# google-deepmind/mujoco_warp

Measured on AMD Instinct MI355X. Metric: env-steps/sec (nworld x steps/s) for humanoid.xml at 8192 worlds, 1/2/4/8 GPUs, higher is better.
Workload: dtype f32; 1 GPU; humanoid.xml, nworld=8192 per GPU, CG solver, Euler, pyramidal, nconmax=24, njmax=64, key 0 + Halton/OU control noise (std 0.01, rate 0.1); nworld_per_gpu=8192, nworld_total=8192, parallelism=worlds sharded over 1 GPU(s), no data-path collective

## Files before the change

### mujoco_warp_amd/csrc/solver_cgp.hpp

```cpp
#pragma once
#include <type_traits>
#include "solver.hpp"
#include "solver_cgw.hpp"

#ifndef MJH_CGP_HOIST
#define MJH_CGP_HOIST 1
#endif
#define CGP_HEAD 32
#define CGP_WORLD 136
template <int NV4>
__host__ __device__ inline int cgp_pool_rows(size_t lds_bytes, int wpb) {
  constexpr int NVR = 4 * NV4, JS = (NV4 & 1) ? NVR : NVR + 4;
  const int words = (int)(lds_bytes / sizeof(float)) - CGP_HEAD - CGP_WORLD * wpb;
  return words <= 0 ? 0 : ((words / JS) & ~3);
}
template <int NV4>
__host__ __device__ inline int cgp_min_rows(int fuse_euler) {
  constexpr int NVR = 4 * NV4, JS = (NV4 & 1) ? NVR : NVR + 4;
  const int words = fuse_euler == 2 ? (6 * 32 + 12 * NV4 + 4 + 32) : (8 * NVR > 32 ? 8 * NVR : 32);
  return (((words + JS - 1) / JS) + 3) & ~3;
}

template <int CTRL>
DEV float qperm(float v) {
  return __int_as_float(__builtin_amdgcn_mov_dpp(__float_as_int(v), CTRL, 0xf, 0xf, true));
}
template <int C>
DEV void fmac_rbc(float& acc, float a, float xs) {
  asm volatile("v_fmac_f32_dpp %0, %1, %2 row_newbcast:%3 row_mask:0xf bank_mask:0xf bound_ctrl:1" : "+v"(acc) : "v"(xs), "v"(a), "n"(C));
}
DEV void dpp_fence(BV& x) { asm volatile("s_nop 4" : "+v"(x.a), "+v"(x.b)); }
template <int C>
DEV void fmac4_rbc(float& s0, float& s1, float a0, float a1, float a2, float a3, float xs) {
  asm volatile(
      "v_fmac_f32_dpp %0, %2, %3 row_newbcast:%7 row_mask:0xf bank_mask:0xf bound_ctrl:1\n\t"
      "v_fmac_f32_dpp %1, %2, %4 row_newbcast:%8 row_mask:0xf bank_mask:0xf bound_ctrl:1\n\t"
      "v_fmac_f32_dpp %0, %2, %5 row_newbcast:%9 row_mask:0xf bank_mask:0xf bound_ctrl:1\n\t"
      "v_fmac_f32_dpp %1, %2, %6 row_newbcast:%10 row_mask:0xf bank_mask:0xf bound_ctrl:1"
      : "+v"(s0), "+v"(s1)
      : "v"(xs), "v"(a0), "v"(a1), "v"(a2), "v"(a3), "n"(C), "n"(C + 1), "n"(C + 2), "n"(C + 3));
}
template <int OFF, int N, int NT>
DEV void fmac_seq(float (&s)[2], const float (&row)[N], float xs) {
  static_assert(NT % 4 == 0, "four terms per asm statement");
  if constexpr (NT >= 4) fmac4_rbc<0>(s[0], s[1], row[OFF], row[OFF + 1], row[OFF + 2], row[OFF + 3], xs);
  if constexpr (NT >= 8) fmac4_rbc<4>(s[0], s[1], row[OFF + 4], row[OFF + 5], row[OFF + 6], row[OFF + 7], xs);
  if constexpr (NT >= 12) fmac4_rbc<8>(s[0], s[1], row[OFF + 8], row[OFF + 9], row[OFF + 10], row[OFF + 11], xs);
  if constexpr (NT >= 16) fmac4_rbc<12>(s[0], s[1], row[OFF + 12], row[OFF + 13], row[OFF + 14], row[OFF + 15], xs);
}
template <int N, int NT>
DEV void fmac_seq2(float (&s)[4], const float (&r0)[N], const float (&r1)[N], float xs) {
  static_assert(NT % 4 == 0, "four terms per asm statement");
  if constexpr (NT >= 4) { fmac4_rbc<0>(s[0], s[1], r0[0], r0[1], r0[2], r0[3], xs); fmac4_rbc<0>(s[2], s[3], r1[0], r1[1], r1[2], r1[3], xs); }
  if constexpr (NT >= 8) { fmac4_rbc<4>(s[0], s[1], r0[4], r0[5], r0[6], r0[7], xs); fmac4_rbc<4>(s[2], s[3], r1[4], r1[5], r1[6], r1[7], xs); }
  if constexpr (NT >= 12) { fmac4_rbc<8>(s[0], s[1], r0[8], r0[9], r0[10], r0[11], xs); fmac4_rbc<8>(s[2], s[3], r1[8], r1[9], r1[10], r1[11], xs); }
  if constexpr (NT >= 16) { fmac4_rbc<12>(s[0], s[1], r0[12], r0[13], r0[14], r0[15], xs); fmac4_rbc<12>(s[2], s[3], r1[12], r1[13], r1[14], r1[15], xs); }
}

template <int NVR, int G>
DEV void invert_rows_b4s(const float (&mrow)[NVR], float (&s)[NVR], float* buf, int lig) {
#pragma unroll
  for (int c = 0; c < NVR; ++c) s[c] = mrow[c];
#pragma unroll
  for (int kb = 0; kb < NVR / 4; ++kb) {
    constexpr int T = 4 * NVR;
    const int k = 4 * kb;
    float* pb = buf + (kb & 1) * T;
    const int q = lig - k;
    if (q >= 0 && q < 4) {
#pragma unroll
      for (int c4 = 0; c4 < NVR / 4; ++c4) *reinterpret_cast<float4*>(pb + q * NVR + 4 * c4) = make_float4(s[4 * c4], s[4 * c4 + 1], s[4 * c4 + 2], s[4 * c4 + 3]);
    }
    gsync();
    const float4 P0 = *reinterpret_cast<const float4*>(pb + k), P1 = *reinterpret_cast<const float4*>(pb + NVR + k),
                 P2 = *reinterpret_cast<const float4*>(pb + 2 * NVR + k), P3 = *reinterpret_cast<const float4*>(pb + 3 * NVR + k);
    const float i0 = 1.0f / P0.x;
    const float l10 = P1.x * i0, l20 = P2.x * i0, l30 = P3.x * i0;
    const float i1 = 1.0f / (P1.y - l10 * P1.x);
    const float t21 = P2.y - l20 * P1.x, t31 = P3.y - l30 * P1.x;
    const float l21 = t21 * i1, l31 = t31 * i1;
    const float i2 = 1.0f / (P2.z - l20 * P2.x - l21 * t21);
    const float t32 = P3.z - l30 * P2.x - l31 * t21;
    const float l32 = t32 * i2;
    const float i3 = 1.0f / (P3.w - l30 * P3.x - l31 * t31 - l32 * t32);
    const float n10 = -l10, n21 = -l21, n32 = -l32;
    const float n20 = -l20 - l21 * n10, n31 = -l31 - l32 * n21;
    const float n30 = -l30 - l31 * n10 - l32 * n20;
    const float e30 = i3 * n30, e31 = i3 * n31, e32 = i3 * n32, e20 = i2 * n20, e21 = i2 * n21, e10 = i1 * n10;
    float Pi[4][4];
    Pi[3][3] = i3;
    Pi[2][3] = Pi[3][2] = e32;
    Pi[1][3] = Pi[3][1] = e31;
    Pi[0][3] = Pi[3][0] = e30;
    Pi[2][2] = i2 + n32 * e32;
    Pi[1][2] = Pi[2][1] = e21 + n31 * e32;
    Pi[0][2] = Pi[2][0] = e20 + n30 * e32;
    Pi[1][1] = i1 + n21 * e21 + n31 * e31;
    Pi[0][1] = Pi[1][0] = e10 + n20 * e21 + n30 * e31;
    Pi[0][0] = i0 + n10 * e10 + n20 * e20 + n30 * e30;
    const bool inb = q >= 0 && q < 4;
    float F[4];
#pragma unroll
    for (int p = 0; p < 4; ++p) {
      const float out = s[k] * Pi[0][p] + s[k + 1] * Pi[1][p] + s[k + 2] * Pi[2][p] + s[k + 3] * Pi[3][p];
      const float own = (q == p ? 1.0f : 0.0f) - (q == 0 ? Pi[0][p] : (q == 1 ? Pi[1][p] : (q == 2 ? Pi[2][p] : Pi[3][p])));
      F[p] = inb ? own : out;
    }
#pragma unroll
    for (int c4 = 0; c4 < NVR / 4; ++c4) {
      if (c4 == kb) continue;
      const float4 r0 = *reinterpret_cast<const float4*>(pb + 4 * c4), r1 = *reinterpret_cast<const float4*>(pb + NVR + 4 * c4),
                   r2 = *reinterpret_cast<const float4*>(pb + 2 * NVR + 4 * c4), r3 = *reinterpret_cast<const float4*>(pb + 3 * NVR + 4 * c4);
      s[4 * c4] -= F[0] * r0.x + F[1] * r1.x + F[2] * r2.x + F[3] * r3.x;
      s[4 * c4 + 1] -= F[0] * r0.y + F[1] * r1.y + F[2] * r2.y + F[3] * r3.y;
      s[4 * c4 + 2] -= F[0] * r0.z + F[1] * r1.z + F[2] * r2.z + F[3] * r3.z;
      s[4 * c4 + 3] -= F[0] * r0.w + F[1] * r1.w + F[2] * r2.w + F[3] * r3.w;
    }
#pragma unroll
    for (int e = 0; e < 4; ++e) s[k + e] = (q == e ? 1.0f : 0.0f) - F[e];
  }
}

template <int NV4>
DEV void solve_cgp_body(const MjhModel& m, const MjhData& d, float* smem, int slot0, int nwb, int pool_rows, int fuse_euler) {
  constexpr int G = 32, NR = 2, NVR = 4 * NV4, JS = (NV4 & 1) ? NVR : NVR + 4, J4 = JS / 4;
  constexpr int NA = NVR < 16 ? NVR : 16, NBX = NVR - NA;
  const int nv = m.nv, nC = m.nC, njmax = d.njmax, nvp = d.nv_pad;
  const int lig = threadIdx.x & (G - 1), gib = threadIdx.x / G;
  const int slot = slot0 + gib;
  const bool valid = gib < nwb && slot < d.nworld;
  int* cnt = reinterpret_cast<int*>(smem);
  int* slotR = reinterpret_cast<int*>(smem) + CGP_HEAD + CGP_WORLD * gib;
  float* fbT = smem + CGP_HEAD + CGP_WORLD * gib + 64;
  float* pool = smem + CGP_HEAD + CGP_WORLD * (blockDim.x / G);
  const bool active = lig < nv;

  const int w = valid ? d.ws_order[slot] : 0;
  const size_t vo = (size_t)w * nv, eo = (size_t)w * njmax;
  int idx[NVR];
  {
    const int nv4r = (nv + 3) >> 2;
    const int4* tab = reinterpret_cast<const int4*>(m.M_dense) + (size_t)(active ? lig : 0) * nv4r;
#pragma unroll
    for (int c4 = 0; c4 < NV4; ++c4) {
      const int4 t4 = c4 < nv4r ? tab[c4] : make_int4(-1, -1, -1, -1);
      idx[4 * c4] = t4.x; idx[4 * c4 + 1] = t4.y; idx[4 * c4 + 2] = t4.z; idx[4 * c4 + 3] = t4.w;
    }
  }
  int nefc = 0, ne = 0, nf = 0, npf = 0;
  int ty[2] = {0, 0};
  if (valid) {
    nefc = min(d.nefc[w], njmax);
    ne = d.ne[w];
    nf = d.nf[w];
    npf = ne + nf + d.nl[w];
#pragma unroll
    for (int k = 0; k < 2; ++k) ty[k] = lig + G * k < njmax ? d.efc_type[eo + lig + G * k] : 0;
  }
  float mrow[NVR];
  {
    const float* Mg = d.M + (size_t)w * nC;
#pragma unroll
    for (int c = 0; c < NVR; ++c) {
      const float v = Mg[idx[c] < 0 ? 0 : idx[c]];
      mrow[c] = active ? (idx[c] < 0 ? 0.0f : v) : (c == lig ? 1.0f : 0.0f);
    }
  }
  const float fs = active ? d.qfrc_smooth[vo + lig] : 0.0f;
  const float qwarm = active ? d.qacc_warmstart[vo + lig] : 0.0f;

  int np = 0, nq = 0, need = 0;
  bool defer = false;
  if (valid) {
    npf = min(npf, nefc);
    bool is6[2];
#pragma unroll
    for (int k = 0; k < 2; ++k) {
      const int r = lig + G * k;
      is6[k] = r >= npf && r < nefc && ty[k] == CT_CONTACT_PYRAMIDAL;
    }
    const unsigned m0 = (unsigned)gballot<G>(is6[0]), m1 = (unsigned)gballot<G>(is6[1]);
    const int n60 = __popc(m0), n6 = n60 + __popc(m1);
    const unsigned below = (1u << lig) - 1u;
#pragma unroll
    for (int k = 0; k < 2; ++k) {
      const int r = lig + G * k;
      const int c6 = k == 0 ? __popc(m0 & below) : n60 + __popc(m1 & below);
      if (r < nefc && r < 64) slotR[is6[k] ? c6 : n6 + r - c6] = r;
      fbT[r] = 0.0f;
    }
    nq = n6 >> 2;
    np = nefc - n6;
    defer = nf > 0 || (n6 & 3) != 0 || nefc > 64;
    need = max((np + 3 * nq + 15) & ~15, cgp_min_rows<NV4>(fuse_euler));
  }
  if (lig == 0 && gib < CGP_HEAD) cnt[gib] = (valid && !defer) ? need : 0;
  __syncthreads();
  int base = 0;
  {
    int acc = 0;
    for (int j = 0; j < nwb; ++j) {
      const int c = cnt[j];
      const bool fits = acc + c <= pool_rows;
      if (j == gib) {
        base = acc;
        if (!fits) defer = true;
      }
      acc += fits ? c : 0;
    }
  }
  if (!valid) return;
  if (defer) {
    if (lig == 0) d.solver_niter[w] = -1;
    return;
  }
  float* Jl = pool + (size_t)base * JS;
  const int nb = np + 3 * nq, nb16 = (nb + 15) & ~15;

  PhaseClock pc(5, lig);
  pc.mark(0);
  const bool warm = !(m.disableflags & DSBL_WARMSTART);
  auto mul_row = [&](const float (&row)[NVR], BV x) __attribute__((always_inline)) {
    float s[2] = {0.0f, 0.0f};
    dpp_fence(x);
    fmac_seq<0, NVR, NA>(s, row, x.a);
    if constexpr (NBX > 0) fmac_seq<NA, NVR, NBX>(s, row, x.b);
    return active ? s[0] + s[1] : 0.0f;
  };
  float h[NVR];
  invert_rows_b4s<NVR, G>(mrow, h, Jl, lig);
  float qs = mul_row(h, bcast_prep(fs));
  {
    const float res = fs - mul_row(mrow, bcast_prep(qs));
    qs += mul_row(h, bcast_prep(active ? res : 0.0f));
  }
  if (active) d.qacc_smooth[vo + lig] = qs;
  float q = active ? (nefc > 0 && warm ? qwarm : qs) : 0.0f;
  pc.mark(1);
  float Ma = mul_row(mrow, bcast_prep(q));
  if (nefc == 0) {
    if (active) {
      d.qacc[vo + lig] = q;
      d.qfrc_constraint[vo + lig] = 0.0f;
      d.efc_Ma[vo + lig] = Ma;
    }
    if (lig == 0) d.solver_niter[w] = 0;
    if (fuse_euler) {
      float qi = q;
      gsync();
      if (fuse_euler == 2) qi = impfast_acc<NV4, G>(m, d, w, lig, active, mrow, Ma, Jl);
      euler_advance<G>(m, d, w, lig, active, qi, Jl + (fuse_euler == 2 ? 6 * G + 12 * NV4 + 4 : 0), q);
    }
    return;
  }

  float rD[NR], rja[NR], rjv[NR];
  int rkind[NR];
  int jro[NR];
  int fbo[NR];
  bool isq[NR];
  int rer[NR];
  const int qd = lig & 3;
#pragma unroll
  for (int k = 0; k < NR; ++k) {
    const int s = lig + G * k;
    const bool has = s < nefc;
    isq[k] = s < 4 * nq;
    const int er = has ? slotR[s] : 0;
    rer[k] = er;
    const int br = isq[k] ? 3 * (s >> 2) + (qd < 3 ? qd : 2) : (has ? s - nq : 0);
    const int bf_ = isq[k] ? (qd < 3 ? 3 * (s >> 2) + qd : -1) : s - nq;
    jro[k] = br * JS;
    fbo[k] = (!has || bf_ < 0) ? 64 : bf_;
    rD[k] = has ? d.efc_D[eo + er] : 0.0f;
    rkind[k] = !has ? 3 : (isq[k] ? 2 : (er < ne ? 0 : 2));
    rjv[k] = 0.0f;
    rja[k] = has ? d.efc_aref[eo + er] : 0.0f;
  }
  gsync();
  {
    const float* Jg = d.efc_J + (size_t)w * d.njmax_pad * nvp;
    const int nvp4 = nvp >> 2;
    for (int it = lig; it < nq * J4; it += G) {
      const int c = it / J4, c4 = it - c * J4;
      float4 r0 = make_float4(0.0f, 0.0f, 0.0f, 0.0f), r1 = r0, r2 = r0, r3 = r0;
      if (c4 < nvp4) {
        const float4* src = reinterpret_cast<const float4*>(Jg + (size_t)slotR[4 * c] * nvp) + c4;
        r0 = src[0]; r1 = src[nvp4]; r2 = src[2 * nvp4]; r3 = src[3 * nvp4];
      }
      float4* dst = reinterpret_cast<float4*>(Jl + (size_t)(3 * c) * JS) + c4;
      dst[0] = make_float4(0.5f * (r0.x + r1.x), 0.5f * (r0.y + r1.y), 0.5f * (r0.z + r1.z), 0.5f * (r0.w + r1.w));
      dst[J4] = make_float4(0.5f * (r0.x - r1.x), 0.5f * (r0.y - r1.y), 0.5f * (r0.z - r1.z), 0.5f * (r0.w - r1.w));
      dst[2 * J4] = make_float4(0.5f * (r2.x - r3.x), 0.5f * (r2.y - r3.y), 0.5f * (r2.z - r3.z), 0.5f * (r2.w - r3.w));
    }
    for (int it = lig; it < (nb16 - 3 * nq) * J4; it += G) {
      const int p = it / J4, c4 = it - p * J4;
      float4 v = make_float4(0.0f, 0.0f, 0.0f, 0.0f);
      if (p < np && c4 < nvp4) v = (reinterpret_cast<const float4*>(Jg + (size_t)slotR[4 * nq + p] * nvp))[c4];
      (reinterpret_cast<float4*>(Jl + (size_t)(3 * nq + p) * JS))[c4] = v;
    }
  }
  gsync();
  auto j_dots = [&](auto nxt, BV x, float (&out)[NR], float* mv) __attribute__((always_inline)) {
    constexpr int NX = decltype(nxt)::value;
    float s[4] = {0.0f, 0.0f, 0.0f, 0.0f};
    float r0[NA], r1[NA];
    auto load_a = [&]() __attribute__((always_inline)) {
#pragma unroll
      for (int c4 = 0; c4 < NA / 4; ++c4) {
        const float4 a4 = *reinterpret_cast<const float4*>(Jl + jro[0] + 4 * c4);
        r0[4 * c4] = a4.x; r0[4 * c4 + 1] = a4.y; r0[4 * c4 + 2] = a4.z; r0[4 * c4 + 3] = a4.w;
        if constexpr (NX > 1) {
          const float4 b4 = *reinterpret_cast<const float4*>(Jl + jro[1] + 4 * c4);
          r1[4 * c4] = b4.x; r1[4 * c4 + 1] = b4.y; r1[4 * c4 + 2] = b4.z; r1[4 * c4 + 3] = b4.w;
        }
      }
    };
    if constexpr (NV4 <= 7) load_a();
    dpp_fence(x);
    if (mv) {
      float t[2] = {0.0f, 0.0f};
      fmac_seq<0, NVR, NA>(t, mrow, x.a);
      if constexpr (NBX > 0) fmac_seq<NA, NVR, NBX>(t, mrow, x.b);
      *mv = active ? t[0] + t[1] : 0.0f;
    }
    if constexpr (NV4 > 7) load_a();
    constexpr int NB_ = NBX > 0 ? NBX : 4;
    float q0[NB_], q1[NB_];
    if constexpr (NBX > 0) {
#pragma unroll
      for (int c4 = 0; c4 < NBX / 4; ++c4) {
        const float4 a4 = *reinterpret_cast<const float4*>(Jl + jro[0] + NA + 4 * c4);
        q0[4 * c4] = a4.x; q0[4 * c4 + 1] = a4.y; q0[4 * c4 + 2] = a4.z; q0[4 * c4 + 3] = a4.w;
        if constexpr (NX > 1) {
          const float4 b4 = *reinterpret_cast<const float4*>(Jl + jro[1] + NA + 4 * c4);
          q1[4 * c4] = b4.x; q1[4 * c4 + 1] = b4.y; q1[4 * c4 + 2] = b4.z; q1[4 * c4 + 3] = b4.w;
        }
      }
    }
    if constexpr (NX > 1) {
      fmac_seq2<NA, NA>(s, r0, r1, x.a);
      if constexpr (NBX > 0) fmac_seq2<NB_, NBX>(s, q0, q1, x.b);
    } else {
      float s2[2] = {0.0f, 0.0f};
      fmac_seq<0, NA, NA>(s2, r0, x.a);
      if constexpr (NBX > 0) fmac_seq<0, NB_, NBX>(s2, q0, x.b);
      s[0] = s2[0];
      s[1] = s2[1];
    }
#pragma unroll
    for (int k = 0; k < NR; ++k) {
      if (k >= NX) {
        out[k] = 0.0f;
        continue;
      }
      const float dt = s[2 * k] + s[2 * k + 1];
      const float dn = qperm<0x00>(dt), d1 = qperm<0x55>(dt), d2 = qperm<0xAA>(dt);
      const float tq = qd < 2 ? d1 : d2;
      const float dq = dn + ((qd & 1) ? -tq : tq);
      out[k] = rkind[k] == 3 ? 0.0f : (isq[k] ? dq : dt);
    }
  };
  {
    float jq[NR];
    j_dots(std::integral_constant<int, NR>{}, bcast_prep(q), jq, nullptr);
#pragma unroll
    for (int k = 0; k < NR; ++k) rja[k] = rkind[k] != 3 ? jq[k] - rja[k] : 0.0f;
  }
  pc.mark(2);
  const float tolerance = bf(m.opt_tolerance, m.opt_tolerance_nb, w, 1)[0];
  const float ls_tolerance = bf(m.opt_ls_tolerance, m.opt_ls_tolerance_nb, w, 1)[0];
  const float meaninertia = bf(m.stat_meaninertia, m.stat_meaninertia_nb, w, 1)[0];
  const float scale = meaninertia * (float)nv;
  const float rscale = 1.0f / scale;
  const int qd4 = lig >> 2;
  const int cq = qd4 < J4 ? qd4 : (qd4 - 4 >= 0 && qd4 - 4 < J4 ? qd4 - 4 : J4 - 1), rg = lig & 3;
  const float* Jq = Jl + 4 * cq + 4 * rg * JS;
  const float *Jq1 = Jq + min(16, nb16 - 16) * JS, *Jq2 = Jq + min(32, nb16 - 16) * JS, *Jq3 = Jq + min(48, nb16 - 16) * JS;

  float grad_dot = 0.0f, search_dot = 0.0f;
  float g = 0.0f, Mg = 0.0f, pg = 0.0f, pMg = 0.0f, srch = 0.0f, qc = 0.0f;
  float cg5[5] = {0.0f, 0.0f, 0.0f, 0.0f, 0.0f};
  int niter = 0;
  const int maxiter = m.iterations, ls_iterations = m.ls_iterations;
  int ovf = 0;
  float improvement = 0.0f;
  const bool short16 = __ballot(nb16 > 16) == 0ull;
  auto iterate = [&](auto nxt) __attribute__((always_inline)) {
  constexpr int NX = decltype(nxt)::value;
  for (;;) {
#if MJH_CGP_HOIST
    const float4 hj0 = *reinterpret_cast<const float4*>(Jq), hj1 = *reinterpret_cast<const float4*>(Jq + JS),
                 hj2 = *reinterpret_cast<const float4*>(Jq + 2 * JS), hj3 = *reinterpret_cast<const float4*>(Jq + 3 * JS);
#endif
#if MJH_CGP_HOIST > 1
    float4 gj0 = make_float4(0.0f, 0.0f, 0.0f, 0.0f), gj1 = gj0, gj2 = gj0, gj3 = gj0;
    if (!(NX == 1 && short16)) {
      gj0 = *reinterpret_cast<const float4*>(Jq1); gj1 = *reinterpret_cast<const float4*>(Jq1 + JS);
      gj2 = *reinterpret_cast<const float4*>(Jq1 + 2 * JS); gj3 = *reinterpret_cast<const float4*>(Jq1 + 3 * JS);
    }
#endif
#pragma unroll
    for (int k = 0; k < NX; ++k) {
      const bool quad = (rkind[k] == 0) | ((rkind[k] == 2) & (rja[k] < 0.0f));
      const float f = quad ? -rD[k] * rja[k] : 0.0f;
      const float a = qperm<0xB1>(f);
      const float sm = f + a, df = f - a;
      const float tot = sm + qperm<0x4E>(sm);
      const float bq = qd == 0 ? tot : (qd == 1 ? -df : df);
      fbT[fbo[k]] = isq[k] ? bq : f;
    }
    gsync();
    {
      float a0 = 0.0f, a1 = 0.0f, a2 = 0.0f, a3 = 0.0f;
      auto batch = [&](int kb, const float* Jb) __attribute__((always_inline)) {
        const float4 f4 = *reinterpret_cast<const float4*>(fbT + 16 * kb + 4 * rg);
        const float4 j0 = *reinterpret_cast<const float4*>(Jb), j1 = *reinterpret_cast<const float4*>(Jb + JS),
                     j2 = *reinterpret_cast<const float4*>(Jb + 2 * JS), j3 = *reinterpret_cast<const float4*>(Jb + 3 * JS);
        a0 += j0.x * f4.x; a1 += j0.y * f4.x; a2 += j0.z * f4.x; a3 += j0.w * f4.x;
        a0 += j1.x * f4.y; a1 += j1.y * f4.y; a2 += j1.z * f4.y; a3 += j1.w * f4.y;
        a0 += j2.x * f4.z; a1 += j2.y * f4.z; a2 += j2.z * f4.z; a3 += j2.w * f4.z;
        a0 += j3.x * f4.w; a1 += j3.y * f4.w; a2 += j3.z * f4.w; a3 += j3.w * f4.w;
      };
#if MJH_CGP_HOIST
      {
        const float4 f4 = *reinterpret_cast<const float4*>(fbT + 4 * rg);
        a0 += hj0.x * f4.x; a1 += hj0.y * f4.x; a2 += hj0.z * f4.x; a3 += hj0.w * f4.x;
        a0 += hj1.x * f4.y; a1 += hj1.y * f4.y; a2 += hj1.z * f4.y; a3 += hj1.w * f4.y;
        a0 += hj2.x * f4.z; a1 += hj2.y * f4.z; a2 += hj2.z * f4.z; a3 += hj2.w * f4.z;
        a0 += hj3.x * f4.w; a1 += hj3.y * f4.w; a2 += hj3.z * f4.w; a3 += hj3.w * f4.w;
      }
#else
      batch(0, Jq);
#endif
#if MJH_CGP_HOIST > 1
      if (!(NX == 1 && short16)) {
        const float4 f4 = *reinterpret_cast<const float4*>(fbT + 16 + 4 * rg);
        a0 += gj0.x * f4.x; a1 += gj0.y * f4.x; a2 += gj0.z * f4.x; a3 += gj0.w * f4.x;
        a0 += gj1.x * f4.y; a1 += gj1.y * f4.y; a2 += gj1.z * f4.y; a3 += gj1.w * f4.y;
        a0 += gj2.x * f4.z; a1 += gj2.y * f4.z; a2 += gj2.z * f4.z; a3 += gj2.w * f4.z;
        a0 += gj3.x * f4.w; a1 += gj3.y * f4.w; a2 += gj3.z * f4.w; a3 += gj3.w * f4.w;
      }
#else
      if (!(NX == 1 && short16)) batch(1, Jq1);
#endif
      if (nb16 > 32) {
        batch(2, Jq2);
        batch(3, Jq3);
      }
      a0 += qperm<0xB1>(a0); a1 += qperm<0xB1>(a1); a2 += qperm<0xB1>(a2); a3 += qperm<0xB1>(a3);
      a0 += qperm<0x4E>(a0); a1 += qperm<0x4E>(a1); a2 += qperm<0x4E>(a2); a3 += qperm<0x4E>(a3);
      const float mine = qd == 0 ? a0 : (qd == 1 ? a1 : (qd == 2 ? a2 : a3));
      qc = active ? mine : 0.0f;
    }
    gsync();
    g = active ? (Ma - fs - qc) : 0.0f;
    pc.mark(3);
    Mg = mul_row(h, bcast_prep(g));
    cg5[0] = g * g; cg5[1] = g * (Mg - pMg); cg5[2] = pg * pMg; cg5[3] = Mg * Mg; cg5[4] = Mg * srch;
    gsum32_valu_n<5>(cg5);
    grad_dot = cg5[0];
    pc.mark(4);
    if (niter == 0) {
      srch = -Mg;
      search_dot = cg5[3];
      pg = g;
      pMg = Mg;
    } else {
      const float imp = improvement * rscale, gradient = sqrtf(grad_dot) * rscale;
      const float beta = fmaxf(0.0f, cg5[1] * __builtin_amdgcn_rcpf(fmaxf(MJ_MINVAL, cg5[2])));
      const bool done = (imp < tolerance) || (gradient < tolerance);
      if (done) break;
      srch = -Mg + beta * srch;
      search_dot = fmaxf(cg5[3] + beta * (beta * search_dot - 2.0f * cg5[4]), 0.0f);
      pg = g;
      pMg = Mg;
      if (niter >= maxiter) {
        ovf |= OVF_ITERATIONS;
        break;
      }
    }
    if (maxiter == 0) break;
    float mvi;
    j_dots(nxt, bcast_prep(srch), rjv, &mvi);
    pc.mark(5);
    const float g1 = srch * (Ma - fs);
    const float gtol = fmaxf(tolerance * ls_tolerance * sqrtf(search_dot) * scale, 1e-6f);
    float alpha = 0.0f;
    improvement = 0.0f;
    bool ls_converged = false;
    if constexpr (NX == NR) {
      line_search_rows<NR, G, false, 1>(rja, rjv, rD, rkind, nullptr, g1, 0.5f * srch * mvi, fabsf(g1), gtol, ls_iterations, alpha, improvement, ls_converged);
    } else {
      const float ja1[1] = {rja[0]}, jv1[1] = {rjv[0]}, D1[1] = {rD[0]};
      const int kind1[1] = {rkind[0]};
      line_search_rows<1, G, false, 1>(ja1, jv1, D1, kind1, nullptr, g1, 0.5f * srch * mvi, fabsf(g1), gtol, ls_iterations, alpha, improvement, ls_converged);
    }
    if (!ls_converged) ovf |= OVF_LS_ITERATIONS;
    pc.mark(6);
    q += alpha * srch;
    Ma += alpha * mvi;
#pragma unroll
    for (int k = 0; k < NX; ++k) rja[k] += alpha * rjv[k];
    ++niter;
    pc.mark(7);
  }
  };
  if (__ballot(nefc > G) == 0ull) iterate(std::integral_constant<int, 1>{});
  else iterate(std::integral_constant<int, NR>{});
  pc.mark(8);
  if (active) {
    d.qacc[vo + lig] = q;
    d.qfrc_constraint[vo + lig] = qc;
    d.efc_Ma[vo + lig] = Ma;
  }
#pragma unroll
  for (int k = 0; k < NR; ++k)
    if (rkind[k] != 3) {
      const bool quad = (rkind[k] == 0) | (rja[k] < 0.0f);
      d.efc_force[eo + rer[k]] = quad ? -rD[k] * rja[k] : 0.0f;
      d.efc_state[eo + rer[k]] = quad ? ST_QUADRATIC : ST_SATISFIED;
    }
  if (lig == 0) {
    d.solver_niter[w] = niter;
    if (ovf) atomicOr(d.overflow + w, ovf);
  }
  if (fuse_euler) {
    gsync();
    float qi = q;
    if (fuse_euler == 2) qi = impfast_acc<NV4, G>(m, d, w, lig, active, mrow, Ma, Jl);
    euler_advance<G>(m, d, w, lig, active, qi, Jl + (fuse_euler == 2 ? 6 * G + 12 * NV4 + 4 : 0), q);
  }
  pc.mark(9);
}
```

Before: 27.79 million env-steps/s.

## Treat joint-limit constraint rows as sparse single-DOF entries in CG solver

```diff
diff --git a/mujoco_warp_amd/csrc/solver_cgp.hpp b/mujoco_warp_amd/csrc/solver_cgp.hpp
--- a/mujoco_warp_amd/csrc/solver_cgp.hpp
+++ b/mujoco_warp_amd/csrc/solver_cgp.hpp
@@ -148,14 +148,22 @@
     }
   }
   int nefc = 0, ne = 0, nf = 0, npf = 0;
-  int ty[2] = {0, 0};
+  int ty[2] = {0, 0}, eid[2] = {0, 0};
   if (valid) {
     nefc = min(d.nefc[w], njmax);
     ne = d.ne[w];
     nf = d.nf[w];
     npf = ne + nf + d.nl[w];
 #pragma unroll
-    for (int k = 0; k < 2; ++k) ty[k] = lig + G * k < njmax ? d.efc_type[eo + lig + G * k] : 0;
+    for (int k = 0; k < 2; ++k) {
+      ty[k] = lig + G * k < njmax ? d.efc_type[eo + lig + G * k] : 0;
+      eid[k] = lig + G * k < njmax ? d.efc_id[eo + lig + G * k] : 0;
+    }
+  }
+  int jinfo = 0;
+  if (lig < m.njnt) {
+    const int jt = m.jnt_type[lig];
+    jinfo = (m.jnt_dofadr[lig] << 1) | ((jt == JNT_SLIDE) | (jt == JNT_HINGE));
   }
   float mrow[NVR];
   {
@@ -173,26 +181,36 @@
   bool defer = false;
   if (valid) {
     npf = min(npf, nefc);
-    bool is6[2];
+    bool is6[2], isl[2];
+    int ldof[2];
 #pragma unroll
     for (int k = 0; k < 2; ++k) {
       const int r = lig + G * k;
       is6[k] = r >= npf && r < nefc && ty[k] == CT_CONTACT_PYRAMIDAL;
+      const int ji = __shfl(jinfo, eid[k] & (G - 1), G);
+      isl[k] = r < nefc && ty[k] == CT_LIMIT_JOINT && (unsigned)eid[k] < (unsigned)min(m.njnt, G) && (ji & 1);
+      ldof[k] = ji >> 1;
     }
     const unsigned m0 = (unsigned)gballot<G>(is6[0]), m1 = (unsigned)gballot<G>(is6[1]);
+    const unsigned l0 = (unsigned)gballot<G>(isl[0]), l1 = (unsigned)gballot<G>(isl[1]);
     const int n60 = __popc(m0), n6 = n60 + __popc(m1);
+    const int nl0 = __popc(l0), nlim = nl0 + __popc(l1);
     const unsigned below = (1u << lig) - 1u;
+    nq = n6 >> 2;
+    np = nefc - n6 - nlim;
 #pragma unroll
     for (int k = 0; k < 2; ++k) {
       const int r = lig + G * k;
       const int c6 = k == 0 ? __popc(m0 & below) : n60 + __popc(m1 & below);
-      if (r < nefc && r < 64) slotR[is6[k] ? c6 : n6 + r - c6] = r;
+      const int cl = k == 0 ? __popc(l0 & below) : nl0 + __popc(l1 & below);
+      if (r < nefc && r < 64) {
+        if (isl[k]) slotR[n6 + np + cl] = r | (ldof[k] << 8);
+        else slotR[is6[k] ? c6 : n6 + r - c6 - cl] = r;
+      }
       fbT[r] = 0.0f;
     }
-    nq = n6 >> 2;
-    np = nefc - n6;
     defer = nf > 0 || (n6 & 3) != 0 || nefc > 64;
-    need = max((np + 3 * nq + 15) & ~15, cgp_min_rows<NV4>(fuse_euler));
+    need = max(nefc > 0 ? max((np + 3 * nq + 15) & ~15, 16) : 0, cgp_min_rows<NV4>(fuse_euler));
   }
   if (lig == 0 && gib < CGP_HEAD) cnt[gib] = (valid && !defer) ? need : 0;
   __syncthreads();
@@ -215,7 +233,7 @@
     return;
   }
   float* Jl = pool + (size_t)base * JS;
-  const int nb = np + 3 * nq, nb16 = (nb + 15) & ~15;
+  const int nb = np + 3 * nq, nb16 = max((nb + 15) & ~15, 16);
 
   PhaseClock pc(5, lig);
   pc.mark(0);
@@ -259,19 +277,24 @@
   int jro[NR];
   int fbo[NR];
   bool isq[NR];
-  int rer[NR];
+  int rerp = 0;
+  bool lneg[NR];
   const int qd = lig & 3;
+  const float* Jg = d.efc_J + (size_t)w * d.njmax_pad * nvp;
 #pragma unroll
   for (int k = 0; k < NR; ++k) {
     const int s = lig + G * k;
     const bool has = s < nefc;
     isq[k] = s < 4 * nq;
-    const int er = has ? slotR[s] : 0;
-    rer[k] = er;
+    const bool lim = has && s >= 4 * nq + np;
+    const int sr = has ? slotR[s] : 0;
+    const int er = sr & 255, ld = (sr >> 8) & (G - 1);
+    rerp |= er << (8 * k);
     const int br = isq[k] ? 3 * (s >> 2) + (qd < 3 ? qd : 2) : (has ? s - nq : 0);
     const int bf_ = isq[k] ? (qd < 3 ? 3 * (s >> 2) + qd : -1) : s - nq;
-    jro[k] = br * JS;
-    fbo[k] = (!has || bf_ < 0) ? 64 : bf_;
+    jro[k] = lim ? (int)(fbT - 32 - Jl) : br * JS;
+    fbo[k] = lim ? ld - 64 : ((!has || bf_ < 0) ? 64 : bf_);
+    lneg[k] = lim && Jg[(size_t)er * nvp + ld] < 0.0f;
     rD[k] = has ? d.efc_D[eo + er] : 0.0f;
     rkind[k] = !has ? 3 : (isq[k] ? 2 : (er < ne ? 0 : 2));
     rjv[k] = 0.0f;
@@ -279,7 +302,6 @@
   }
   gsync();
   {
-    const float* Jg = d.efc_J + (size_t)w * d.njmax_pad * nvp;
     const int nvp4 = nvp >> 2;
     for (int it = lig; it < nq * J4; it += G) {
       const int c = it / J4, c4 = it - c * J4;
@@ -301,10 +323,19 @@
     }
   }
   gsync();
-  auto j_dots = [&](auto nxt, BV x, float (&out)[NR], float* mv) __attribute__((always_inline)) {
+  float* fline = fbT - 64;
+  fline[lig] = 0.0f;
+  fline[G + lig] = 0.0f;
+  const int xsrc = threadIdx.x & 32;
+  auto j_dots = [&](auto nxt, float xd, BV x, float (&out)[NR], float* mv) __attribute__((always_inline)) {
     constexpr int NX = decltype(nxt)::value;
     float s[4] = {0.0f, 0.0f, 0.0f, 0.0f};
     float r0[NA], r1[NA];
+#pragma unroll
+    for (int k = 0; k < NX; ++k) {
+      const float xl = __int_as_float(__builtin_amdgcn_ds_bpermute(((fbo[k] & (G - 1)) | xsrc) << 2, __float_as_int(xd)));
+      s[2 * k] = fbo[k] < 0 ? (lneg[k] ? -xl : xl) : 0.0f;
+    }
     auto load_a = [&]() __attribute__((always_inline)) {
 #pragma unroll
       for (int c4 = 0; c4 < NA / 4; ++c4) {
@@ -342,7 +373,7 @@
       fmac_seq2<NA, NA>(s, r0, r1, x.a);
       if constexpr (NBX > 0) fmac_seq2<NB_, NBX>(s, q0, q1, x.b);
     } else {
-      float s2[2] = {0.0f, 0.0f};
+      float s2[2] = {s[0], 0.0f};
       fmac_seq<0, NA, NA>(s2, r0, x.a);
       if constexpr (NBX > 0) fmac_seq<0, NB_, NBX>(s2, q0, x.b);
       s[0] = s2[0];
@@ -363,7 +394,7 @@
   };
   {
     float jq[NR];
-    j_dots(std::integral_constant<int, NR>{}, bcast_prep(q), jq, nullptr);
+    j_dots(std::integral_constant<int, NR>{}, q, bcast_prep(q), jq, nullptr);
 #pragma unroll
     for (int k = 0; k < NR; ++k) rja[k] = rkind[k] != 3 ? jq[k] - rja[k] : 0.0f;
   }
@@ -408,7 +439,7 @@
       const float sm = f + a, df = f - a;
       const float tot = sm + qperm<0x4E>(sm);
       const float bq = qd == 0 ? tot : (qd == 1 ? -df : df);
-      fbT[fbo[k]] = isq[k] ? bq : f;
+      fbT[fbo[k]] = isq[k] ? bq : (lneg[k] ? -f : f);
     }
     gsync();
     {
@@ -444,10 +475,12 @@
 #else
       if (!(NX == 1 && short16)) batch(1, Jq1);
 #endif
+      const float fl = fline[lig];
       if (nb16 > 32) {
         batch(2, Jq2);
         batch(3, Jq3);
       }
+      a0 += qd == 0 ? fl : 0.0f; a1 += qd == 1 ? fl : 0.0f; a2 += qd == 2 ? fl : 0.0f; a3 += qd == 3 ? fl : 0.0f;
       a0 += qperm<0xB1>(a0); a1 += qperm<0xB1>(a1); a2 += qperm<0xB1>(a2); a3 += qperm<0xB1>(a3);
       a0 += qperm<0x4E>(a0); a1 += qperm<0x4E>(a1); a2 += qperm<0x4E>(a2); a3 += qperm<0x4E>(a3);
       const float mine = qd == 0 ? a0 : (qd == 1 ? a1 : (qd == 2 ? a2 : a3));
@@ -482,7 +515,7 @@
     }
     if (maxiter == 0) break;
     float mvi;
-    j_dots(nxt, bcast_prep(srch), rjv, &mvi);
+    j_dots(nxt, srch, bcast_prep(srch), rjv, &mvi);
     pc.mark(5);
     const float g1 = srch * (Ma - fs);
     const float gtol = fmaxf(tolerance * ls_tolerance * sqrtf(search_dot) * scale, 1e-6f);
@@ -509,27 +542,31 @@
   if (__ballot(nefc > G) == 0ull) iterate(std::integral_constant<int, 1>{});
   else iterate(std::integral_constant<int, NR>{});
   pc.mark(8);
+  int wo = w, rp = rerp;
+  asm volatile("" : "+v"(wo), "+v"(rp));
+  const size_t vo2 = (size_t)wo * nv, eo2 = (size_t)wo * njmax;
   if (active) {
-    d.qacc[vo + lig] = q;
-    d.qfrc_constraint[vo + lig] = qc;
-    d.efc_Ma[vo + lig] = Ma;
+    d.qacc[vo2 + lig] = q;
+    d.qfrc_constraint[vo2 + lig] = qc;
+    d.efc_Ma[vo2 + lig] = Ma;
   }
 #pragma unroll
   for (int k = 0; k < NR; ++k)
     if (rkind[k] != 3) {
       const bool quad = (rkind[k] == 0) | (rja[k] < 0.0f);
-      d.efc_force[eo + rer[k]] = quad ? -rD[k] * rja[k] : 0.0f;
-      d.efc_state[eo + rer[k]] = quad ? ST_QUADRATIC : ST_SATISFIED;
+      const int er = (rp >> (8 * k)) & 255;
+      d.efc_force[eo2 + er] = quad ? -rD[k] * rja[k] : 0.0f;
+      d.efc_state[eo2 + er] = quad ? ST_QUADRATIC : ST_SATISFIED;
     }
   if (lig == 0) {
-    d.solver_niter[w] = niter;
-    if (ovf) atomicOr(d.overflow + w, ovf);
+    d.solver_niter[wo] = niter;
+    if (ovf) atomicOr(d.overflow + wo, ovf);
   }
   if (fuse_euler) {
     gsync();
     float qi = q;
-    if (fuse_euler == 2) qi = impfast_acc<NV4, G>(m, d, w, lig, active, mrow, Ma, Jl);
-    euler_advance<G>(m, d, w, lig, active, qi, Jl + (fuse_euler == 2 ? 6 * G + 12 * NV4 + 4 : 0), q);
+    if (fuse_euler == 2) qi = impfast_acc<NV4, G>(m, d, wo, lig, active, mrow, Ma, Jl);
+    euler_advance<G>(m, d, wo, lig, active, qi, Jl + (fuse_euler == 2 ? 6 * G + 12 * NV4 + 4 : 0), q);
   }
   pc.mark(9);
 }
```

New measurement: 27.79 million env-steps/s. About the same (-0.0%).
